# vfdev-5/interpolate-antialiasing

Measured on AMD Instinct MI355X. Metric: Mpix/s (input pixels) antialiased bilinear 438x906->196x320, uint8 channels_last, PIL-exact, higher is better.
Workload: dtype u8; 1 GPU; uint8 channels_last [1024,3,438,906]->[196,320] bilinear antialias per GPU (BASELINE configs[1] batched), Pillow-exact integer arithmetic; batch_per_gpu=1024, global_batch=1024, variant=fused_u8_nhwc_pil_v3, parallelism=batch-shard x1, lib=interpolate_antialiasing_amd/csrc/libaa_interp.so

## Files before the change

interpolate_antialiasing_amd/csrc/aa_fused_u8_v3_impl.h:

```cpp

#pragma once
#include <math.h>
#include <stdio.h>
#include <stdlib.h>

#include <type_traits>

#include "aa_alpha.h"
#include "aa_plan.h"

#ifndef AA_V3_ABL
#define AA_V3_ABL 0
#endif

#ifndef AA_V3_AUX
#define AA_V3_AUX 0
#endif

#ifndef AA_V3_PRIO
#define AA_V3_PRIO 0
#endif
#ifndef AA_V3_DMA_EARLY
#define AA_V3_DMA_EARLY 0
#endif

#ifndef AA_V3_BURST
#define AA_V3_BURST 1
#endif

#ifndef AA_V3_F32OUT_AUX
#define AA_V3_F32OUT_AUX 0
#endif

#ifndef AA_V3_FLT_FAST
#define AA_V3_FLT_FAST 0
#endif

#ifndef AA_V3_UNALIGNED
#define AA_V3_UNALIGNED 0
#endif

struct FusedU8V3Params {
  int H, W, oH, oW;
  int ksize_w, ksize_h;
  int ybands, nstrips;
  int strips_per_block;
  int strip_w;
  int nseg;
  int seg_bytes;
  int sc_off;
  int gather_off;
  int in_mis;
  unsigned long long img_in_bytes, img_out_bytes, total_in_bytes, total_out_bytes;
  long long n_images;
  int spb_forced;
  int outm, normalize, cin;
  float mean[4], std[4];
  unsigned row_pitch;
  int fast;
  int byte_store;
  unsigned long long plane_in_bytes, plane_out_bytes;
  long long pl_planes;
  int out16, pair_store;
};

namespace {

typedef __attribute__((address_space(3))) void lds_void;

#ifndef AA_V3_STORE_AUX
#define AA_V3_STORE_AUX 2
#endif
constexpr int kStoreAuxInterleaved = AA_V3_STORE_AUX;



__device__ inline unsigned pack4_clip8(int a0, int a1, int a2, int a3) {
  unsigned d;
  asm("v_ashr_pk_u8_i32 %0, %1, %2, 22\n\tv_ashr_pk_u8_i32 %0, %3, %4, 22 op_sel:[0,0,0,1]"
      : "=&v"(d)
      : "v"(a0), "v"(a1), "v"(a2), "v"(a3));
  return d;
}

__device__ inline unsigned pack2_bf16(float lo, float hi) {
  unsigned d;
  asm("v_cvt_pk_bf16_f32 %0, %1, %2" : "=v"(d) : "v"(lo), "v"(hi));
  return d;
}
__device__ inline unsigned pack2_f16(float lo, float hi) {
  typedef _Float16 half2_t __attribute__((ext_vector_type(2)));
  const half2_t t = {(_Float16)lo, (_Float16)hi};
  return __builtin_bit_cast(unsigned, t);
}

__device__ inline float right_neighbour(float x) {
  return __int_as_float(__builtin_amdgcn_update_dpp(__float_as_int(x), __float_as_int(x), 0xF5 , 0xF, 0xF, false));
}

__device__ inline int clip8_int(int acc) {
  acc >>= 22;
  return acc < 0 ? 0 : (acc > 255 ? 255 : acc);
}

__device__ inline void wait_vmcnt(int n) {
  if (n >= 12) { asm volatile("s_waitcnt vmcnt(12)" ::: "memory"); return; }
  if (n >= 8) { asm volatile("s_waitcnt vmcnt(8)" ::: "memory"); return; }
  if (n >= 6) { asm volatile("s_waitcnt vmcnt(6)" ::: "memory"); return; }
  if (n >= 4) { asm volatile("s_waitcnt vmcnt(4)" ::: "memory"); return; }
  if (n >= 3) { asm volatile("s_waitcnt vmcnt(3)" ::: "memory"); return; }
  if (n >= 2) { asm volatile("s_waitcnt vmcnt(2)" ::: "memory"); return; }
  if (n >= 1) { asm volatile("s_waitcnt vmcnt(1)" ::: "memory"); return; }
  asm volatile("s_waitcnt vmcnt(0)" ::: "memory");
}

#ifndef AA_V3_WAVES_PER_EU
#define AA_V3_WAVES_PER_EU 0
#endif
#if AA_V3_WAVES_PER_EU
#define AA_V3_OCC __attribute__((amdgpu_waves_per_eu(AA_V3_WAVES_PER_EU, AA_V3_WAVES_PER_EU)))
#else
#define AA_V3_OCC
#endif
template <int C, int TW, int G, bool TWO_DMA, int MAXC, bool NONNEG, bool PERIODIC, bool FLT = false, int UPK = 0, int PL = 0, int SP = 1,
          bool ALPHA = false, bool O16 = false>
__global__ void __launch_bounds__(512) AA_V3_OCC
fused_u8_nhwc_v3_kernel(const uint8_t *__restrict__ in, uint8_t *__restrict__ out, const char *__restrict__ tab_w,
                        const char *__restrict__ tab_h, const FusedU8V3Params p) {
  static_assert(PL == 0 || (PL == C && !PERIODIC && UPK == 0 && !TWO_DMA), "plane groups: shrinking heights, fixed stage layout");
  static_assert(SP == 1 || (SP == 4 && !FLT && !PERIODIC && UPK == 0 && PL == 0), "split windows: integer arithmetic, shrinking heights");
  static_assert(!ALPHA || (C == 4 && !FLT && PL == 0), "premultiplied alpha: Pillow arithmetic, 4 interleaved channels");
  static_assert(!O16 || (FLT && SP == 1), "16-bit float output: float arithmetic");
  constexpr int PLN = PL > 0 ? PL : 1;
  constexpr int CB = PL > 0 ? 1 : C;
  constexpr int NV1 = (CB * TW + 3) / 4;
  constexpr int ND1 = NV1 + 1;
  constexpr int NV = PLN * NV1, ND = PLN * ND1;
  struct SA { unsigned s[PLN]; };
  constexpr int PL_SLOT = 1024, PL_PIECES = 21, PL_PLANE = PL_PIECES * 16;
  extern __shared__ __attribute__((aligned(16))) uint8_t lds[];

  const int lane = threadIdx.x & 63;
  const int wv = __builtin_amdgcn_readfirstlane(threadIdx.x >> 6);
  const int sgroups = (p.nstrips + p.strips_per_block - 1) / p.strips_per_block;
  const int xcd = blockIdx.x & 7, k = blockIdx.x >> 3;
  const int strip = (k % sgroups) * p.strips_per_block + wv;
  const long long grp = (long long)(k / sgroups) * 8 + xcd;
  if (grp >= p.n_images * p.ybands) return;
  if (strip >= p.nstrips) return;
  const bool full_group = (k % sgroups + 1) * p.strips_per_block <= p.nstrips;
  const int yb = (int)(grp % p.ybands);
  const int n = (int)(grp / p.ybands);
  const int ox0 = strip * p.strip_w;
  const int bw = min(p.strip_w, p.oW - ox0);
  const int oy0 = (int)((long long)yb * p.oH / p.ybands);
  const int oy1 = (int)((long long)(yb + 1) * p.oH / p.ybands);

  const int32_t *__restrict__ xmin_w = (const int32_t *)(tab_w + aa_table_xmin_off());
  const int32_t *__restrict__ xsize_w = (const int32_t *)(tab_w + aa_table_xsize_off(p.oW));
  const int32_t *__restrict__ kw = (const int32_t *)(tab_w + aa_table_w_off(p.oW));
  const int32_t *__restrict__ ymin_h = (const int32_t *)(tab_h + aa_table_xmin_off());
  const int32_t *__restrict__ ysize_h = (const int32_t *)(tab_h + aa_table_xsize_off(p.oH));
  const int32_t *__restrict__ sc_rec = (const int32_t *)(tab_h + p.sc_off);
  const int32_t *__restrict__ g_rec = (const int32_t *)(tab_h + p.gather_off);

  const int r_begin = __builtin_amdgcn_readfirstlane(ymin_h[oy0]);
  const int ylm = __builtin_amdgcn_readfirstlane(ymin_h[oy1 - 1]);
  const int yls = __builtin_amdgcn_readfirstlane(ysize_h[oy1 - 1]);
  const int r_stop = ylm + (yls > 1 ? yls : 1);
  const int n_rows = r_stop - r_begin;
  const int n_groups = (n_rows + G - 1) / G;

  const int sp_px = SP > 1 ? lane / SP : lane;
  const int sp_part = SP > 1 ? lane % SP : 0;
  const bool active = sp_px < bw;
  const int ox = ox0 + (active ? sp_px : 0);
  const int xm = xmin_w[ox];
  int xs = xsize_w[ox];
  xs = xs > 1 ? xs : 1;
  int lead = xm + TW * SP - p.W;
  lead = lead > 0 ? lead : 0;
  const int start = xm - lead + sp_part * TW;
  const int acc_init = (SP > 1 && sp_part != 0) ? 0 : 1 << 21;
  int wreg[TW];
#pragma unroll
  for (int j = 0; j < TW; j++) {
    const int src = sp_part * TW + j - lead;
    int w = (src >= 0 && src < xs && src < p.ksize_w) ? kw[(size_t)ox * p.ksize_w + src] : 0;
    wreg[j] = FLT ? w : (w << 8) >> 8;
  }
  asm volatile("s_waitcnt vmcnt(0)" ::: "memory");
  const int seg_first = __builtin_amdgcn_readfirstlane(start * CB);
  const int c_l = start * CB - seg_first;

  const unsigned long long img_off = (unsigned long long)p.in_mis + (unsigned long long)n * p.img_in_bytes;
  const unsigned long long base_off = img_off & ~15ull;
  unsigned long long remaining = p.total_in_bytes - base_off;
  if constexpr (PL == 0) remaining = (remaining + 3ull) & ~3ull;
  if (remaining > 0xFFFFFFFCull) remaining = 0xFFFFFFFCull;
  const __amdgpu_buffer_rsrc_t rsrc =
      __builtin_amdgcn_make_buffer_rsrc((void *)(in + base_off), 0, (unsigned)remaining, 0x00020000);
  const unsigned row_bytes = p.row_pitch;
  const int lds_base = PL > 0 ? wv * G * PL_SLOT : wv * G * p.seg_bytes;
  const unsigned lane_lds = (unsigned)(lds_base + c_l);
  unsigned pl_voff = 0;
  bool pl_dma_lane = false;
  if constexpr (PL > 0) {
    const int pc = lane / PL_PIECES, piece = lane - pc * PL_PIECES;
    pl_voff = (unsigned)pc * (unsigned)p.plane_in_bytes + (unsigned)piece * 16u;
    pl_dma_lane = pc < PL && piece < p.nseg;
  }
  const bool dma_lane0 = PL > 0 ? pl_dma_lane : lane < p.nseg;
  const bool dma_lane1 = lane + 64 < p.nseg;
  constexpr int dma_per_row = TWO_DMA ? 2 : 1;
  const unsigned voff = (unsigned)lane * 16u;

  const unsigned long long out_off = (unsigned long long)n * p.img_out_bytes;
  unsigned long long out_rem = p.total_out_bytes - out_off;
  if (out_rem > 0xFFFFFFFFull) out_rem = 0xFFFFFFFFull;
  const __amdgpu_buffer_rsrc_t orsrc = __builtin_amdgcn_make_buffer_rsrc((void *)(out + out_off), 0, (unsigned)out_rem, 0x00020000);
  const unsigned out_row_bytes = (unsigned)p.oW * CB;
  const int pl_valid = PL > 0 ? (int)(p.pl_planes - (long long)n * PL < PL ? p.pl_planes - (long long)n * PL : PL) : C;
  float nm_mean[C], nm_std[C];
#pragma unroll
  for (int c = 0; c < C; c++) {
    const int ch = PL > 0 ? (int)(((long long)n * PL + c) % (p.cin > 0 ? p.cin : 1))
                          : (C == 1 ? (int)(n % (p.cin > 0 ? p.cin : 1)) : c);
    nm_mean[c] = FLT ? p.mean[ch & 3] : 0.f;
    nm_std[c] = FLT ? p.std[ch & 3] : 1.f;
  }
  unsigned store_voff;
  bool store_lane;
  unsigned perm_sel = 0;
  if constexpr (PL > 0) {
    store_voff = (unsigned)(ox0 + lane);
    store_lane = ((lane & 3) == 0) && ((lane | 3) < bw);
  } else if constexpr (C == 3) {
    const int q = lane & 3;
    store_voff = (unsigned)(ox0 * 3 + (lane >> 2) * 12 + q * 4);
    store_lane = (q != 3) && ((lane | 3) < bw);
    perm_sel = q == 0 ? 0x04020100u : (q == 1 ? 0x05040201u : 0x06050402u);
  } else if constexpr (C == 1) {
    store_voff = (unsigned)(ox0 + lane);
    store_lane = ((lane & 3) == 0) && ((lane | 3) < bw);
  } else {
    store_voff = (unsigned)((ox0 + lane) * 4);
    store_lane = active;
  }

  unsigned a = (unsigned)(img_off - base_off) + (unsigned)seg_first + (unsigned)r_begin * row_bytes;

  int A[MAXC][C];
#pragma unroll
  for (int k = 0; k < MAXC; k++)
#pragma unroll
    for (int c = 0; c < C; c++) A[k][c] = FLT ? 0 : 1 << 21;
  int o_base = oy0;

  constexpr int RK = UPK > 0 ? UPK : 1;
  int ring[RK][C];
#pragma unroll
  for (int k = 0; k < RK; k++)
#pragma unroll
    for (int c = 0; c < C; c++) ring[k][c] = 0;
  int vm_issued = 0, idxv = 0;

  auto dma = [&](unsigned a_row, int slot) {
    if (AA_V3_ABL == 4) return;
    if constexpr (UPK > 0) {
      vm_issued += TWO_DMA ? 2 : 1;
      idxv = (lane == slot) ? vm_issued : idxv;
    }
    if (AA_V3_PRIO) __builtin_amdgcn_s_setprio(3);
    const unsigned soff = AA_V3_ABL == 7 ? (a_row & 0x3F0u) : (a_row & ~15u);
    const int dst = lds_base + slot * (PL > 0 ? PL_SLOT : p.seg_bytes);
    if constexpr (PL > 0) {
      if (dma_lane0) __builtin_amdgcn_raw_ptr_buffer_load_lds(rsrc, (lds_void *)(lds + dst), 16, pl_voff, a_row, 0, AA_V3_AUX);
      if (AA_V3_PRIO) __builtin_amdgcn_s_setprio(0);
      return;
    }
    if (dma_lane0) __builtin_amdgcn_raw_ptr_buffer_load_lds(rsrc, (lds_void *)(lds + dst), 16, voff, soff, 0, AA_V3_AUX);
    if constexpr (TWO_DMA) {
      if (dma_lane1)
        __builtin_amdgcn_raw_ptr_buffer_load_lds(rsrc, (lds_void *)(lds + dst + 1024), 16, voff + 1024, soff, 0, AA_V3_AUX);
    }
    if (AA_V3_PRIO) __builtin_amdgcn_s_setprio(0);
  };
  unsigned slot_ra[G];
  unsigned slot_ph[G];
#pragma unroll
  for (int j = 0; j < G; j++) {
    const unsigned ph = (a + (unsigned)j * row_bytes) & 15u;
    slot_ph[j] = (unsigned)(j * p.seg_bytes) + ph;
    slot_ra[j] = (lane_lds + slot_ph[j]) & ~3u;
  }
  auto fetch = [&](unsigned a_row, int slot, unsigned (&d)[ND], bool tables = true) -> SA {
    SA r;
    unsigned sa, ra;
    if (AA_V3_ABL == 6) { for (int c = 0; c < PLN; c++) r.s[c] = 0; return r; }
    if constexpr (PL > 0) {
      const __attribute__((address_space(3))) unsigned *al = (const __attribute__((address_space(3))) unsigned *)(uintptr_t)(lane_lds & ~3u);
#pragma unroll
      for (int c = 0; c < PL; c++) {
#pragma unroll
        for (int k = 0; k < ND1; k++) d[c * ND1 + k] = al[(slot * PL_SLOT + c * PL_PLANE) / 4 + k];
        r.s[c] = lane_lds;
      }
      return r;
    }
    if (PERIODIC && tables) {
      sa = lane_lds + slot_ph[slot];
      ra = slot_ra[slot];
    } else {
      sa = lane_lds + (unsigned)(slot * p.seg_bytes) + (a_row & 15u);
      ra = sa & ~3u;
    }
    if constexpr (AA_V3_UNALIGNED) {
      typedef unsigned u32_any __attribute__((aligned(1)));
      const __attribute__((address_space(3))) u32_any *ul = (const __attribute__((address_space(3))) u32_any *)(uintptr_t)sa;
#pragma unroll
      for (int k = 0; k < NV; k++) d[k] = ul[k];
      d[ND - 1] = 0;
      r.s[0] = sa;
      return r;
    }
    const __attribute__((address_space(3))) unsigned *al = (const __attribute__((address_space(3))) unsigned *)(uintptr_t)ra;
#pragma unroll
    for (int k = 0; k < ND; k++) d[k] = al[k];
    r.s[0] = sa;
    return r;
  };
  struct Scatter { int first; int cc; int w[MAXC]; };
  auto load_scatter = [&](int r) -> Scatter {
    Scatter s;
    if constexpr (UPK > 0) {
      s.first = 0; s.cc = 0;
#pragma unroll
      for (int k = 0; k < MAXC; k++) s.w[k] = 0;
      return s;
    }
    const int32_t *rec = (const int32_t *)((const char *)sc_rec + (unsigned)r * 32u);
    s.first = __builtin_amdgcn_readfirstlane(rec[0]);
    s.cc = __builtin_amdgcn_readfirstlane(rec[1]);
#pragma unroll
    for (int k = 0; k < MAXC; k++) s.w[k] = __builtin_amdgcn_readfirstlane(rec[2 + k]);
    return s;
  };
  auto trunc8 = [&](int bits) -> unsigned {
    float a = __int_as_float(bits);
    a = a < 0.f ? 0.f : (a > 255.f ? 255.f : a);
    return (unsigned)(int)a;
  };
  const int emit_path = __builtin_amdgcn_readfirstlane(
      (FLT && p.outm != 0) ? (O16 ? (1 | (p.pair_store ? 2 : 0) | (p.out16 == 2 ? 4 : 0) | ((C == 1 || p.outm == 1) ? 8 : 0)) : 1) : (p.byte_store ? 2 : 0));
  auto emit = [&](int oy) {
    if constexpr (ALPHA) {
      const int al = clip8_int(A[0][3]);
#pragma unroll
      for (int c = 0; c < 3; c++) A[0][c] = aa_unpremul8(clip8_int(A[0][c]), al) << 22;
      A[0][3] = al << 22;
    }
    if constexpr (FLT) {
      if constexpr (O16) {
        if (emit_path & 1) {
          int lane_o = lane;
          asm volatile("" : "+v"(lane_o));
          auto pack2 = [&](float lo, float hi) -> unsigned { return (emit_path & 4) ? pack2_bf16(lo, hi) : pack2_f16(lo, hi); };
          auto value = [&](int c) -> float {
            const float x = __int_as_float(A[0][c]);
            return p.normalize ? (x - nm_mean[c]) / nm_std[c] : x;
          };
          const bool pairs = (emit_path & 2) != 0;
          const bool all = lane_o < bw, st = all && (!pairs || (lane_o & 1) == 0);
          if (emit_path & 8) {
            if constexpr (UPK > 0) vm_issued += C;
            const unsigned fv = (unsigned)(ox0 + lane_o) * 2u;
#pragma unroll
            for (int c = 0; c < C; c++) {
              const unsigned fs = ((unsigned)c * (unsigned)p.oH + (unsigned)oy) * (unsigned)p.oW * 2u;
              const float x = value(c);
              const unsigned d = pack2(x, right_neighbour(x));
              if (pairs) {
                if (st && (PL == 0 || c < pl_valid)) __builtin_amdgcn_raw_buffer_store_b32(d, orsrc, fv, fs, AA_V3_F32OUT_AUX);
              } else {
                if (st && (PL == 0 || c < pl_valid)) __builtin_amdgcn_raw_buffer_store_b16((unsigned short)d, orsrc, fv, fs, AA_V3_F32OUT_AUX);
              }
            }
          } else if constexpr (C > 1) {
            const unsigned fv = (unsigned)(ox0 + lane_o) * (unsigned)(2 * C), fs = (unsigned)oy * (unsigned)p.oW * (unsigned)(2 * C);
            float x[C];
#pragma unroll
            for (int c = 0; c < C; c++) x[c] = value(c);
            unsigned d[3];
            if constexpr (C == 3) {
              d[2] = pack2(right_neighbour(x[1]), right_neighbour(x[2]));
              d[1] = pack2(x[2], right_neighbour(x[0]));
              d[0] = pack2(x[0], x[1]);
            } else {
              d[0] = pack2(x[0], x[1]);
              d[1] = pack2(x[2], x[C - 1]);
              d[2] = 0;
            }
            if (!pairs) {
              if constexpr (UPK > 0) vm_issued += C;
#pragma unroll
              for (int c = 0; c < C; c++)
                if (all) __builtin_amdgcn_raw_buffer_store_b16((unsigned short)(d[c >> 1] >> (16 * (c & 1))), orsrc, fv + 2u * (unsigned)c, fs, AA_V3_F32OUT_AUX);
            } else {
              if constexpr (UPK > 0) vm_issued += 1;
              if constexpr (C == 3) {
                typedef unsigned u32x3 __attribute__((ext_vector_type(3)));
                const u32x3 t = {d[0], d[1], d[2]};
                if (st) __builtin_amdgcn_raw_buffer_store_b96(t, orsrc, fv, fs, AA_V3_F32OUT_AUX);
              } else {
                typedef unsigned u32x2 __attribute__((ext_vector_type(2)));
                const u32x2 t = {d[0], d[1]};
                if (all) __builtin_amdgcn_raw_buffer_store_b64(t, orsrc, fv, fs, AA_V3_F32OUT_AUX);
              }
            }
          }
        }
      } else
      if (emit_path == 1) {
        float v[C];
        int lane_o = lane;
        asm volatile("" : "+v"(lane_o));
#pragma unroll
        for (int c = 0; c < C; c++) {
          v[c] = __int_as_float(A[0][c]);
          if (p.normalize) v[c] = (v[c] - nm_mean[c]) / nm_std[c];
        }
        if (p.outm == 1) {
          if constexpr (UPK > 0) vm_issued += C;
#pragma unroll
          for (int c = 0; c < C; c++)
            if (active && (PL == 0 || c < pl_valid))
              __builtin_amdgcn_raw_buffer_store_b32(__float_as_uint(v[c]), orsrc, (unsigned)(ox0 + lane_o) * 4u,
                                                    ((unsigned)c * (unsigned)p.oH + (unsigned)oy) * (unsigned)p.oW * 4u, AA_V3_F32OUT_AUX);
        } else {
          if constexpr (UPK > 0) vm_issued += 1;
          const unsigned fv = (unsigned)(ox0 + lane_o) * (unsigned)(4 * C), fs = (unsigned)oy * (unsigned)p.oW * (unsigned)(4 * C);
          if constexpr (C == 3) {
            typedef unsigned u32x3 __attribute__((ext_vector_type(3)));
            const u32x3 t = {__float_as_uint(v[0]), __float_as_uint(v[1]), __float_as_uint(v[2])};
            if (active) __builtin_amdgcn_raw_buffer_store_b96(t, orsrc, fv, fs, AA_V3_F32OUT_AUX);
          } else if constexpr (C == 4) {
            typedef unsigned u32x4 __attribute__((ext_vector_type(4)));
            const u32x4 t = {__float_as_uint(v[0]), __float_as_uint(v[1]), __float_as_uint(v[2]), __float_as_uint(v[3])};
            if (active) __builtin_amdgcn_raw_buffer_store_b128(t, orsrc, fv, fs, AA_V3_F32OUT_AUX);
          } else {
            if (active) __builtin_amdgcn_raw_buffer_store_b32(__float_as_uint(v[0]), orsrc, fv, fs, AA_V3_F32OUT_AUX);
          }
        }
      }
    }
    if (emit_path == 2) {
      int lane_o = lane;
      asm volatile("" : "+v"(lane_o));
      const int px_o = SP > 1 ? lane_o / SP : lane_o;
      const unsigned bv = (unsigned)((ox0 + px_o) * CB);
      const bool act = px_o < bw && (SP == 1 || (lane_o % SP) == 0);
      if constexpr (UPK > 0) vm_issued += C;
#pragma unroll
      for (int c = 0; c < C; c++) {
        const unsigned b = FLT ? trunc8(A[0][c]) : (unsigned)clip8_int(A[0][c]);
        if constexpr (PL > 0) {
          if (act && c < pl_valid) __builtin_amdgcn_raw_buffer_store_b8((unsigned char)b, orsrc, bv, (unsigned)c * (unsigned)p.plane_out_bytes + (unsigned)oy * out_row_bytes, 0);
        } else {
          if (act) __builtin_amdgcn_raw_buffer_store_b8((unsigned char)b, orsrc, bv + c, (unsigned)oy * out_row_bytes, 0);
        }
      }
    }
    if constexpr (UPK > 0) {
      if (emit_path == 0) vm_issued += 1;
    }
    if (emit_path != 0) {
    } else if constexpr (PL > 0) {
      const unsigned t = FLT ? (trunc8(A[0][0]) | (trunc8(A[0][1]) << 8) | (trunc8(A[0][PL > 2 ? 2 : 1]) << 16))
                             : pack4_clip8(A[0][0], A[0][1], A[0][PL > 2 ? 2 : 1], A[0][PL - 1]);
      const unsigned nb = (unsigned)__builtin_amdgcn_update_dpp(0, (int)t, 0xF5 , 0xF, 0xF, false);
#pragma unroll
      for (int c = 0; c < PL; c++) {
        const unsigned pair = __builtin_amdgcn_perm(nb, t, 0x0c0c0000u | (unsigned)((4 + c) << 8) | (unsigned)c);
        const unsigned hi = (unsigned)__builtin_amdgcn_update_dpp(0, (int)pair, 0xAA , 0xF, 0xF, false);
        const unsigned dw = __builtin_amdgcn_perm(hi, pair, 0x05040100u);
        if (store_lane && c < pl_valid) __builtin_amdgcn_raw_buffer_store_b32(dw, orsrc, store_voff, (unsigned)c * (unsigned)p.plane_out_bytes + (unsigned)oy * out_row_bytes, 0);
      }
    } else if constexpr (C == 3) {
      const unsigned t = FLT ? (trunc8(A[0][0]) | (trunc8(A[0][1]) << 8) | (trunc8(A[0][2]) << 16))
                             : pack4_clip8(A[0][0], A[0][1], A[0][2], A[0][2]);
      const unsigned nb = (unsigned)__builtin_amdgcn_update_dpp(0, (int)t, 0xF9 , 0xF, 0xF, false);
      const unsigned dw = __builtin_amdgcn_perm(nb, t, perm_sel);
      if (store_lane && (AA_V3_ABL != 1 || dw == 0x12345678u))
        __builtin_amdgcn_raw_buffer_store_b32(dw, orsrc, store_voff, AA_V3_ABL == 9 ? 0u : (unsigned)oy * out_row_bytes, C == 1 ? 0 : kStoreAuxInterleaved);
    } else if constexpr (C == 1) {
      const unsigned t = FLT ? trunc8(A[0][0]) * 0x01010101u : pack4_clip8(A[0][0], A[0][0], A[0][0], A[0][0]);
      const unsigned n1 = (unsigned)__builtin_amdgcn_update_dpp(0, (int)t, 0x55 , 0xF, 0xF, false);
      const unsigned n2 = (unsigned)__builtin_amdgcn_update_dpp(0, (int)t, 0xAA , 0xF, 0xF, false);
      const unsigned n3 = (unsigned)__builtin_amdgcn_update_dpp(0, (int)t, 0xFF , 0xF, 0xF, false);
      const unsigned dw = (t & 0x000000ffu) | (n1 & 0x0000ff00u) | (n2 & 0x00ff0000u) | (n3 & 0xff000000u);
      if (store_lane) __builtin_amdgcn_raw_buffer_store_b32(dw, orsrc, store_voff, (unsigned)oy * out_row_bytes, C == 1 ? 0 : kStoreAuxInterleaved);
    } else {
      const unsigned dw = FLT ? (trunc8(A[0][0]) | (trunc8(A[0][1]) << 8) | (trunc8(A[0][2]) << 16) | (trunc8(A[0][C - 1]) << 24))
                              : pack4_clip8(A[0][0], A[0][1], A[0][2], A[0][C - 1]);
      if (store_lane) __builtin_amdgcn_raw_buffer_store_b32(dw, orsrc, store_voff, (unsigned)oy * out_row_bytes, C == 1 ? 0 : kStoreAuxInterleaved);
    }
#pragma unroll
    for (int k = 0; k + 1 < MAXC; k++)
#pragma unroll
      for (int c = 0; c < C; c++) A[k][c] = A[k + 1][c];
#pragma unroll
    for (int c = 0; c < C; c++) A[MAXC - 1][c] = FLT ? 0 : 1 << 21;
  };
  struct GRow { int m; int s; int w[RK]; };
  auto load_grow = [&](int oy) -> GRow {
    GRow gr;
    const int o = oy < p.oH ? oy : p.oH - 1;
    const int32_t *rec = (const int32_t *)((const char *)g_rec + (unsigned)o * 32u);
    gr.m = __builtin_amdgcn_readfirstlane(rec[0]);
    gr.s = __builtin_amdgcn_readfirstlane(rec[1]);
#pragma unroll
    for (int k = 0; k < RK; k++) gr.w[k] = __builtin_amdgcn_readfirstlane(rec[2 + (k < 6 ? k : 5)]);
    return gr;
  };
  GRow g_cur, g_nxt;
  if constexpr (UPK > 0) {
    g_cur = load_grow(oy0);
    g_nxt = load_grow(oy0 + 1);
  }
  int r = r_begin;
  auto realign = [&](const unsigned (&d)[ND], const SA &sa, unsigned (&v)[NV]) {
#pragma unroll
    for (int c = 0; c < PLN; c++)
#pragma unroll
      for (int k = 0; k < NV1; k++)
        v[c * NV1 + k] = AA_V3_UNALIGNED ? d[c * ND1 + k] : __builtin_amdgcn_alignbyte(d[c * ND1 + k + 1], d[c * ND1 + k], sa.s[c]);
  };
  bool steady = false;
  auto row_step = [&](const unsigned (&v)[NV], const Scatter &sc, auto steady_tag) {
    constexpr bool STEADY = decltype(steady_tag)::value;
    if (AA_V3_ABL == 6) return;
    int h[C];
    if constexpr (FLT) {
      float accf[C];
#pragma unroll
      for (int j = 0; j < TW; j++) {
#pragma unroll
        for (int c = 0; c < C; c++) {
          const int bi = PL > 0 ? c * (4 * NV1) + j : j * C + c;
          const float px = (float)((v[bi >> 2] >> (8 * (bi & 3))) & 0xffu);
          if constexpr (AA_V3_FLT_FAST != 0) {
            accf[c] = j == 0 ? px * __int_as_float(wreg[j]) : __builtin_fmaf(px, __int_as_float(wreg[j]), accf[c]);
            continue;
          }
          const float prod = px * __int_as_float(wreg[j]);
          accf[c] = j == 0 ? prod : accf[c] + prod;
        }
      }
#pragma unroll
      for (int c = 0; c < C; c++) h[c] = __float_as_int(accf[c]);
    } else {
      int acc[C];
#pragma unroll
      for (int c = 0; c < C; c++) acc[c] = AA_V3_ABL == 5 ? (int)v[c] : (SP > 1 ? acc_init : 1 << 21);
#pragma unroll
      for (int j = 0; j < (AA_V3_ABL == 5 ? 0 : TW); j++) {
#pragma unroll
        for (int c = 0; c < C; c++) {
          const int bi = PL > 0 ? c * (4 * NV1) + j : j * C + c;
          int px = (int)((v[bi >> 2] >> (8 * (bi & 3))) & 0xffu);
          if constexpr (ALPHA) {
            if (c < 3) px = aa_premul8(px, (int)(v[j] >> 24));
          }
          acc[c] += px * wreg[j];
        }
      }
      if constexpr (SP > 1) {
#pragma unroll
        for (int c = 0; c < C; c++) {
          acc[c] += __builtin_amdgcn_update_dpp(0, acc[c], 0xB1 , 0xF, 0xF, false);
          acc[c] += __builtin_amdgcn_update_dpp(0, acc[c], 0x4E , 0xF, 0xF, false);
        }
      }
#pragma unroll
      for (int c = 0; c < C; c++) h[c] = NONNEG ? (int)((unsigned)acc[c] >> 22) : clip8_int(acc[c]);
    }
    if constexpr (UPK > 0) {
#pragma unroll
      for (int k = 0; k + 1 < RK; k++)
#pragma unroll
        for (int c = 0; c < C; c++) ring[k][c] = ring[k + 1][c];
#pragma unroll
      for (int c = 0; c < C; c++) ring[RK - 1][c] = h[c];
      while (o_base < oy1) {
        int gs = g_cur.s > 1 ? g_cur.s : 1;
        if (g_cur.m + gs != r + 1) break;
        gs = gs < RK ? gs : RK;
#pragma unroll
        for (int ss = 1; ss <= RK; ss++) {
          if (gs == ss) {
#pragma unroll
            for (int c = 0; c < C; c++) {
              int acc;
              if constexpr (FLT) {
                float f = __int_as_float(ring[RK - ss][c]) * __int_as_float(g_cur.w[0]);
#pragma unroll
                for (int k2 = 1; k2 < ss; k2++) f = f + __int_as_float(ring[RK - ss + k2][c]) * __int_as_float(g_cur.w[k2]);
                acc = __float_as_int(f);
              } else {
                acc = (1 << 21) + __mul24(ring[RK - ss][c], g_cur.w[0]);
#pragma unroll
                for (int k2 = 1; k2 < ss; k2++) acc += __mul24(ring[RK - ss + k2][c], g_cur.w[k2]);
              }
              A[0][c] = acc;
            }
          }
        }
        emit(o_base);
        o_base++;
        g_cur = g_nxt;
        g_nxt = load_grow(o_base + 1);
      }
      return;
    }
    auto vmac = [&](int a, int hv, int w) -> int {
      if constexpr (FLT && AA_V3_FLT_FAST != 0) return __float_as_int(__builtin_fmaf(__int_as_float(hv), __int_as_float(w), __int_as_float(a)));
      else if constexpr (FLT) return __float_as_int(__int_as_float(a) + __int_as_float(hv) * __int_as_float(w));
      else return a + __mul24(hv, w);
    };
    const int idx0 = sc.first - o_base;
    if constexpr (STEADY) {
#pragma unroll
      for (int k = 0; k < MAXC; k++) {
        if (k >= 2 && k >= (sc.cc & 0xFFFF)) break;
#pragma unroll
        for (int c = 0; c < C; c++) A[k][c] = vmac(A[k][c], h[c], sc.w[k]);
      }
    } else if (__builtin_expect(idx0 == 0, 1)) {
      steady = true;
#pragma unroll
      for (int k = 0; k < MAXC; k++) {
        if (k >= 2 && k >= (sc.cc & 0xFFFF)) break;
#pragma unroll
        for (int c = 0; c < C; c++) A[k][c] = vmac(A[k][c], h[c], sc.w[k]);
      }
    } else if (idx0 < 0 && idx0 > -MAXC) {
#pragma unroll
      for (int s = 1; s < MAXC; s++) {
        if (idx0 == -s) {
#pragma unroll
          for (int k = s; k < MAXC; k++)
#pragma unroll
            for (int c = 0; c < C; c++) A[k - s][c] = vmac(A[k - s][c], h[c], sc.w[k]);
        }
      }
    }
    const int sc_end = sc.first + (sc.cc >> 16);
    const int e_end = sc_end < oy1 ? sc_end : oy1;
    while (o_base < e_end) {
      emit(o_base);
      o_base++;
    }
  };

  const int pl_fix_row = (PL > 0 && (long long)n + 1 == p.n_images) ? p.H - 1 : -1;
  auto pl_patch_last = [&](int slot) {
    if constexpr (PL > 0) {
      const int q = p.W - 3 + lane;
      const int lpos = q - seg_first;
      if (lane < 3 && q >= 0 && lpos >= 0 && lpos < p.nseg * 16) {
        const uint8_t b = in[img_off + (unsigned long long)(pl_valid - 1) * p.plane_in_bytes + (unsigned long long)(p.H - 1) * row_bytes + (unsigned)q];
        lds[lds_base + slot * PL_SLOT + (pl_valid - 1) * PL_PLANE + lpos] = b;
      }
      asm volatile("s_waitcnt vmcnt(0) lgkmcnt(0)" ::: "memory");
    }
  };

  for (int i = 0; i < G; i++)
    if (i < n_rows) dma(a + (unsigned)i * row_bytes, i);
  unsigned d0[ND], d1[ND];
  SA sa0 = {}, sa1 = {};
  Scatter sc0 = load_scatter(r_begin), sc1 = sc0;
  {
    const int younger = (n_rows < G ? n_rows : G) - 1;
    wait_vmcnt(younger * dma_per_row);
    if (PL > 0 && r_begin == pl_fix_row) pl_patch_last(0);
    sa0 = fetch(a, 0, d0, false);
  }
  for (int g = 0; g < n_groups; g++) {
    const int x0 = g * G;
    auto unrolled_group = [&](auto steady_tag) {
      if (full_group) __builtin_amdgcn_s_barrier();
#pragma unroll
      for (int i = 0; i < G; i++) {
        if (AA_V3_ABL != 2) asm volatile("s_waitcnt vmcnt(%0)" ::"n"(dma_per_row * (G - 2 - (i % AA_V3_BURST))) : "memory");
        unsigned v[NV];
        if ((i & 1) == 0) {
          realign(d0, sa0, v);
          __builtin_amdgcn_sched_barrier(0);
          sc1 = load_scatter(r + 1);
          sa1 = fetch(a + row_bytes, (i + 1) % G, d1);
          __builtin_amdgcn_sched_barrier(0);
          if (AA_V3_DMA_EARLY) { dma(a + (unsigned)G * row_bytes, i); __builtin_amdgcn_sched_barrier(0); }
          row_step(v, sc0, steady_tag);
        } else {
          realign(d1, sa1, v);
          __builtin_amdgcn_sched_barrier(0);
          sc0 = load_scatter(r + 1);
          sa0 = fetch(a + row_bytes, (i + 1) % G, d0);
          __builtin_amdgcn_sched_barrier(0);
          if (AA_V3_DMA_EARLY) { dma(a + (unsigned)G * row_bytes, i); __builtin_amdgcn_sched_barrier(0); }
          row_step(v, sc1, steady_tag);
        }
        if (!AA_V3_DMA_EARLY) {
          if constexpr (AA_V3_BURST == 1) {
            dma(a + (unsigned)G * row_bytes, i);
          } else if ((i % AA_V3_BURST) == AA_V3_BURST - 1) {
#pragma unroll
            for (int b = AA_V3_BURST - 1; b >= 0; b--) dma(a + (unsigned)(G - b) * row_bytes, i - b);
          }
        }
        a += row_bytes;
        r++;
        __builtin_amdgcn_sched_barrier(0);
      }
    };
    if (UPK == 0 && x0 + 2 * G <= n_rows) {
      if (steady) unrolled_group(std::true_type{});
      else unrolled_group(std::false_type{});
    } else {
      for (int i = 0; i < G; i++) {
        const int x = x0 + i;
        if (x >= n_rows) break;
        if (x + 1 < n_rows) {
          if constexpr (UPK > 0) {
            const int my_idx = __builtin_amdgcn_readlane(idxv, __builtin_amdgcn_readfirstlane((i + 1) % G));
            wait_vmcnt(vm_issued - my_idx);
          } else {
            int younger = n_rows - 1 - (x + 1);
            younger = younger < G - 2 ? younger : G - 2;
            wait_vmcnt(younger * dma_per_row);
          }
          if (PL > 0 && r + 1 == pl_fix_row) pl_patch_last((i + 1) % G);
          if ((i & 1) == 0) { sc1 = load_scatter(r + 1); sa1 = fetch(a + row_bytes, (i + 1) % G, d1, false); }
          else { sc0 = load_scatter(r + 1); sa0 = fetch(a + row_bytes, (i + 1) % G, d0, false); }
        }
        unsigned v[NV];
        if ((i & 1) == 0) { realign(d0, sa0, v); row_step(v, sc0, std::false_type{}); }
        else { realign(d1, sa1, v); row_step(v, sc1, std::false_type{}); }
        if (x + G < n_rows) dma(a + (unsigned)G * row_bytes, i);
        a += row_bytes;
        r++;
      }
    }
  }
}

int pick_ybands(int64_t items_per_band, double slots, int taps_h, int64_t H, int64_t oH) {
  const int64_t max_yb = oH / 8 > 1 ? oH / 8 : 1;
  int64_t ybands = 1;
  double best = 1e30;
  for (int64_t yb = 1; yb <= max_yb && yb <= 64; yb++) {
    const double rounds = (double)items_per_band * yb / slots;
    const double eff = rounds / ceil(rounds);
    const double halo = 1.0 + (double)(yb - 1) * taps_h / (double)H;
    const double cost = halo / eff;
    if (cost < best - 1e-9) {
      best = cost;
      ybands = yb;
    }
  }
  if (const char *e = aa_knob("AA_FUSED_YBANDS")) {
    const int64_t v = atoll(e);
    if (v >= 1 && v <= max_yb) ybands = v;
  }
  return (int)ybands;
}

template <int C, int TW, int G, int MAXC, bool TWO, bool NONNEG, bool PERIODIC, bool FLT = false, int UPK = 0, int PL = 0, int SP = 1,
          bool ALPHA = false, bool O16 = false>
int launch_k(FusedU8V3Params p, const AAProblem &q, size_t lds) {
  auto kern = fused_u8_nhwc_v3_kernel<C, TW, G, TWO, MAXC, NONNEG, PERIODIC, FLT, UPK, PL, SP, ALPHA, O16>;
  auto resident = [&](int s) {
    int nb = aa_resident_blocks(kern, 64 * s, lds * s);
    if (nb <= 0) nb = 16 / s;
    return nb < 1 ? 1 : nb;
  };
  int spb = p.strips_per_block;
  if (spb > 1 && !p.spb_forced && resident(1) > resident(spb) * spb) spb = 1;
  p.strips_per_block = spb;
  const int sgroups = (p.nstrips + spb - 1) / spb;
  const size_t lds_blk = lds * spb;
  const int taps_h = q.ah.max_taps > 0 ? q.ah.max_taps : q.ah.ksize;
  p.ybands = pick_ybands(p.n_images * sgroups, (double)aa_device_cu_count() * resident(spb), taps_h, q.H, q.oH);
  if (aa_knob("AA_V3_DEBUG"))
    fprintf(stderr, "[aa v3] strips %d spb %d (resident(1) %d, resident(%d) %d) ybands %d lds/strip %zu images %lld\n", p.nstrips, spb,
            resident(1), p.nstrips <= 8 ? p.nstrips : 4, resident(p.nstrips <= 8 ? p.nstrips : 4), p.ybands, lds, (long long)p.n_images);
  const int64_t groups8 = (p.n_images * (int64_t)p.ybands + 7) / 8 * 8;
  const int64_t grid = groups8 * sgroups;
  if (grid > 0x7FFFFFFF) return 0;
  hipLaunchKernelGGL(kern, dim3((unsigned)grid), dim3(64 * spb), lds_blk,
                     q.stream, (const uint8_t *)q.in - p.in_mis, (uint8_t *)q.out, (const char *)q.aw.table_dev,
                     (const char *)q.ah.table_dev, p);
  AA_HIP_CHECK_LAUNCH();
  return 1;
}

int round_tw(int taps) {
  const int opts[] = {2, 4, 6, 8, 12, 16, 24, 34};
  for (int o : opts)
    if (taps <= o) return o;
  return 0;
}

}

enum V3Route {
#define V3_ROUTE(route, ...) V3_##route,
#include "aa_fused_u8_v3_list.h"
};
enum V3Arith { V3_PIL = 1, V3_FLT = 2, V3_BOTH = 3 };
constexpr bool v3_route_has_out16(int route) { return route == V3_NARROW || route == V3_UP || route == V3_PLANES; }
```

Baseline: 1.405 million Mpix/s.

## Replace accumulator sliding with parity-indexed double accumulators and dword-only emit path

Result: slower. 1.379 million Mpix/s (-1.8%).

```diff
diff --git a/interpolate_antialiasing_amd/csrc/aa_fused_u8_v3_impl.h b/interpolate_antialiasing_amd/csrc/aa_fused_u8_v3_impl.h
--- a/interpolate_antialiasing_amd/csrc/aa_fused_u8_v3_impl.h
+++ b/interpolate_antialiasing_amd/csrc/aa_fused_u8_v3_impl.h
@@ -38,6 +38,10 @@
 
 #ifndef AA_V3_UNALIGNED
 #define AA_V3_UNALIGNED 0
+#endif
+
+#ifndef AA_V3_NOSLIDE
+#define AA_V3_NOSLIDE 1
 #endif
 
 struct FusedU8V3Params {
@@ -98,6 +102,10 @@
   return __int_as_float(__builtin_amdgcn_update_dpp(__float_as_int(x), __float_as_int(x), 0xF5 , 0xF, 0xF, false));
 }
 
+template <int QUAD_PERM> __device__ inline unsigned quad_move(unsigned x) {
+  return (unsigned)__builtin_amdgcn_mov_dpp((int)x, QUAD_PERM, 0xF, 0xF, true);
+}
+
 __device__ inline int clip8_int(int acc) {
   acc >>= 22;
   return acc < 0 ? 0 : (acc > 255 ? 255 : acc);
@@ -353,21 +361,27 @@
   };
   const int emit_path = __builtin_amdgcn_readfirstlane(
       (FLT && p.outm != 0) ? (O16 ? (1 | (p.pair_store ? 2 : 0) | (p.out16 == 2 ? 4 : 0) | ((C == 1 || p.outm == 1) ? 8 : 0)) : 1) : (p.byte_store ? 2 : 0));
-  auto emit = [&](int oy) {
+  constexpr bool NS = AA_V3_NOSLIDE != 0 && MAXC == 2 && !FLT && UPK == 0 && PL == 0 && SP == 1 && !ALPHA;
+  int par = 0;
+  auto emit = [&](int oy, auto set_tag, auto dw_tag) {
+    constexpr int S = decltype(set_tag)::value;
+    constexpr bool DW = decltype(dw_tag)::value;
+    static_assert(S == 0 || NS, "only the no-slide form emits from a set other than 0");
+    static_assert(!DW || !FLT, "the dword-only form belongs to the Pillow-arithmetic kernels");
     if constexpr (ALPHA) {
-      const int al = clip8_int(A[0][3]);
-#pragma unroll
-      for (int c = 0; c < 3; c++) A[0][c] = aa_unpremul8(clip8_int(A[0][c]), al) << 22;
-      A[0][3] = al << 22;
-    }
-    if constexpr (FLT) {
+      const int al = clip8_int(A[S][3]);
+#pragma unroll
+      for (int c = 0; c < 3; c++) A[S][c] = aa_unpremul8(clip8_int(A[S][c]), al) << 22;
+      A[S][3] = al << 22;
+    }
+    if constexpr (FLT && !DW) {
       if constexpr (O16) {
         if (emit_path & 1) {
           int lane_o = lane;
           asm volatile("" : "+v"(lane_o));
           auto pack2 = [&](float lo, float hi) -> unsigned { return (emit_path & 4) ? pack2_bf16(lo, hi) : pack2_f16(lo, hi); };
           auto value = [&](int c) -> float {
-            const float x = __int_as_float(A[0][c]);
+            const float x = __int_as_float(A[S][c]);
             return p.normalize ? (x - nm_mean[c]) / nm_std[c] : x;
           };
           const bool pairs = (emit_path & 2) != 0;
@@ -427,7 +441,7 @@
         asm volatile("" : "+v"(lane_o));
 #pragma unroll
         for (int c = 0; c < C; c++) {
-          v[c] = __int_as_float(A[0][c]);
+          v[c] = __int_as_float(A[S][c]);
           if (p.normalize) v[c] = (v[c] - nm_mean[c]) / nm_std[c];
         }
         if (p.outm == 1) {
@@ -454,7 +468,7 @@
         }
       }
     }
-    if (emit_path == 2) {
+    if (!DW && emit_path == 2) {
       int lane_o = lane;
       asm volatile("" : "+v"(lane_o));
       const int px_o = SP > 1 ? lane_o / SP : lane_o;
@@ -463,7 +477,7 @@
       if constexpr (UPK > 0) vm_issued += C;
 #pragma unroll
       for (int c = 0; c < C; c++) {
-        const unsigned b = FLT ? trunc8(A[0][c]) : (unsigned)clip8_int(A[0][c]);
+        const unsigned b = FLT ? trunc8(A[S][c]) : (unsigned)clip8_int(A[S][c]);
         if constexpr (PL > 0) {
           if (act && c < pl_valid) __builtin_amdgcn_raw_buffer_store_b8((unsigned char)b, orsrc, bv, (unsigned)c * (unsigned)p.plane_out_bytes + (unsigned)oy * out_row_bytes, 0);
         } else {
@@ -474,43 +488,48 @@
     if constexpr (UPK > 0) {
       if (emit_path == 0) vm_issued += 1;
     }
-    if (emit_path != 0) {
+    if (!DW && emit_path != 0) {
     } else if constexpr (PL > 0) {
-      const unsigned t = FLT ? (trunc8(A[0][0]) | (trunc8(A[0][1]) << 8) | (trunc8(A[0][PL > 2 ? 2 : 1]) << 16))
-                             : pack4_clip8(A[0][0], A[0][1], A[0][PL > 2 ? 2 : 1], A[0][PL - 1]);
-      const unsigned nb = (unsigned)__builtin_amdgcn_update_dpp(0, (int)t, 0xF5 , 0xF, 0xF, false);
+      const unsigned t = FLT ? (trunc8(A[S][0]) | (trunc8(A[S][1]) << 8) | (trunc8(A[S][PL > 2 ? 2 : 1]) << 16))
+                             : pack4_clip8(A[S][0], A[S][1], A[S][PL > 2 ? 2 : 1], A[S][PL - 1]);
+      const unsigned nb = quad_move<0xF5>(t) ;
 #pragma unroll
       for (int c = 0; c < PL; c++) {
         const unsigned pair = __builtin_amdgcn_perm(nb, t, 0x0c0c0000u | (unsigned)((4 + c) << 8) | (unsigned)c);
-        const unsigned hi = (unsigned)__builtin_amdgcn_update_dpp(0, (int)pair, 0xAA , 0xF, 0xF, false);
+        const unsigned hi = quad_move<0xAA>(pair) ;
         const unsigned dw = __builtin_amdgcn_perm(hi, pair, 0x05040100u);
         if (store_lane && c < pl_valid) __builtin_amdgcn_raw_buffer_store_b32(dw, orsrc, store_voff, (unsigned)c * (unsigned)p.plane_out_bytes + (unsigned)oy * out_row_bytes, 0);
       }
     } else if constexpr (C == 3) {
-      const unsigned t = FLT ? (trunc8(A[0][0]) | (trunc8(A[0][1]) << 8) | (trunc8(A[0][2]) << 16))
-                             : pack4_clip8(A[0][0], A[0][1], A[0][2], A[0][2]);
-      const unsigned nb = (unsigned)__builtin_amdgcn_update_dpp(0, (int)t, 0xF9 , 0xF, 0xF, false);
+      const unsigned t = FLT ? (trunc8(A[S][0]) | (trunc8(A[S][1]) << 8) | (trunc8(A[S][2]) << 16))
+                             : pack4_clip8(A[S][0], A[S][1], A[S][2], A[S][2]);
+      const unsigned nb = quad_move<0xF9>(t) ;
       const unsigned dw = __builtin_amdgcn_perm(nb, t, perm_sel);
       if (store_lane && (AA_V3_ABL != 1 || dw == 0x12345678u))
         __builtin_amdgcn_raw_buffer_store_b32(dw, orsrc, store_voff, AA_V3_ABL == 9 ? 0u : (unsigned)oy * out_row_bytes, C == 1 ? 0 : kStoreAuxInterleaved);
     } else if constexpr (C == 1) {
-      const unsigned t = FLT ? trunc8(A[0][0]) * 0x01010101u : pack4_clip8(A[0][0], A[0][0], A[0][0], A[0][0]);
-      const unsigned n1 = (unsigned)__builtin_amdgcn_update_dpp(0, (int)t, 0x55 , 0xF, 0xF, false);
-      const unsigned n2 = (unsigned)__builtin_amdgcn_update_dpp(0, (int)t, 0xAA , 0xF, 0xF, false);
-      const unsigned n3 = (unsigned)__builtin_amdgcn_update_dpp(0, (int)t, 0xFF , 0xF, 0xF, false);
+      const unsigned t = FLT ? trunc8(A[S][0]) * 0x01010101u : pack4_clip8(A[S][0], A[S][0], A[S][0], A[S][0]);
+      const unsigned n1 = quad_move<0x55>(t) ;
+      const unsigned n2 = quad_move<0xAA>(t) ;
+      const unsigned n3 = quad_move<0xFF>(t) ;
       const unsigned dw = (t & 0x000000ffu) | (n1 & 0x0000ff00u) | (n2 & 0x00ff0000u) | (n3 & 0xff000000u);
       if (store_lane) __builtin_amdgcn_raw_buffer_store_b32(dw, orsrc, store_voff, (unsigned)oy * out_row_bytes, C == 1 ? 0 : kStoreAuxInterleaved);
     } else {
-      const unsigned dw = FLT ? (trunc8(A[0][0]) | (trunc8(A[0][1]) << 8) | (trunc8(A[0][2]) << 16) | (trunc8(A[0][C - 1]) << 24))
-                              : pack4_clip8(A[0][0], A[0][1], A[0][2], A[0][C - 1]);
+      const unsigned dw = FLT ? (trunc8(A[S][0]) | (trunc8(A[S][1]) << 8) | (trunc8(A[S][2]) << 16) | (trunc8(A[S][C - 1]) << 24))
+                              : pack4_clip8(A[S][0], A[S][1], A[S][2], A[S][C - 1]);
       if (store_lane) __builtin_amdgcn_raw_buffer_store_b32(dw, orsrc, store_voff, (unsigned)oy * out_row_bytes, C == 1 ? 0 : kStoreAuxInterleaved);
     }
-#pragma unroll
-    for (int k = 0; k + 1 < MAXC; k++)
-#pragma unroll
-      for (int c = 0; c < C; c++) A[k][c] = A[k + 1][c];
-#pragma unroll
-    for (int c = 0; c < C; c++) A[MAXC - 1][c] = FLT ? 0 : 1 << 21;
+    if constexpr (NS) {
+#pragma unroll
+      for (int c = 0; c < C; c++) A[S][c] = 1 << 21;
+    } else {
+#pragma unroll
+      for (int k = 0; k + 1 < MAXC; k++)
+#pragma unroll
+        for (int c = 0; c < C; c++) A[k][c] = A[k + 1][c];
+#pragma unroll
+      for (int c = 0; c < C; c++) A[MAXC - 1][c] = FLT ? 0 : 1 << 21;
+    }
   };
   struct GRow { int m; int s; int w[RK]; };
   auto load_grow = [&](int oy) -> GRow {
@@ -537,7 +556,7 @@
         v[c * NV1 + k] = AA_V3_UNALIGNED ? d[c * ND1 + k] : __builtin_amdgcn_alignbyte(d[c * ND1 + k + 1], d[c * ND1 + k], sa.s[c]);
   };
   bool steady = false;
-  auto row_step = [&](const unsigned (&v)[NV], const Scatter &sc, auto steady_tag) {
+  auto row_step = [&](const unsigned (&v)[NV], const Scatter &sc, auto steady_tag, auto dw_tag) {
     constexpr bool STEADY = decltype(steady_tag)::value;
     if (AA_V3_ABL == 6) return;
     int h[C];
@@ -616,7 +635,7 @@
             }
           }
         }
-        emit(o_base);
+        emit(o_base, std::integral_constant<int, 0>{}, dw_tag);
         o_base++;
         g_cur = g_nxt;
         g_nxt = load_grow(o_base + 1);
@@ -629,7 +648,19 @@
       else return a + __mul24(hv, w);
     };
     const int idx0 = sc.first - o_base;
-    if constexpr (STEADY) {
+    if constexpr (NS) {
+      int lw0 = sc.w[0], lw1 = sc.w[1];
+      if constexpr (!STEADY) {
+        if (idx0 == 0) steady = true;
+        lw0 = idx0 == 0 ? sc.w[0] : (idx0 == -1 ? sc.w[1] : 0);
+        lw1 = idx0 == 0 ? sc.w[1] : 0;
+      }
+      const int pw0 = par ? lw1 : lw0, pw1 = par ? lw0 : lw1;
+#pragma unroll
+      for (int c = 0; c < C; c++) A[0][c] = vmac(A[0][c], h[c], pw0);
+#pragma unroll
+      for (int c = 0; c < C; c++) A[1][c] = vmac(A[1][c], h[c], pw1);
+    } else if constexpr (STEADY) {
 #pragma unroll
       for (int k = 0; k < MAXC; k++) {
         if (k >= 2 && k >= (sc.cc & 0xFFFF)) break;
@@ -657,9 +688,20 @@
     }
     const int sc_end = sc.first + (sc.cc >> 16);
     const int e_end = sc_end < oy1 ? sc_end : oy1;
-    while (o_base < e_end) {
-      emit(o_base);
-      o_base++;
+    if constexpr (NS) {
+#pragma unroll
+      for (int k = 0; k < MAXC; k++) {
+        if (o_base >= e_end) break;
+        if (par) emit(o_base, std::integral_constant<int, 1>{}, dw_tag);
+        else emit(o_base, std::integral_constant<int, 0>{}, dw_tag);
+        par ^= 1;
+        o_base++;
+      }
+    } else {
+      while (o_base < e_end) {
+        emit(o_base, std::integral_constant<int, 0>{}, dw_tag);
+        o_base++;
+      }
     }
   };
 
@@ -689,7 +731,7 @@
   }
   for (int g = 0; g < n_groups; g++) {
     const int x0 = g * G;
-    auto unrolled_group = [&](auto steady_tag) {
+    auto unrolled_group = [&](auto steady_tag, auto dw_tag) {
       if (full_group) __builtin_amdgcn_s_barrier();
 #pragma unroll
       for (int i = 0; i < G; i++) {
@@ -702,7 +744,7 @@
           sa1 = fetch(a + row_bytes, (i + 1) % G, d1);
           __builtin_amdgcn_sched_barrier(0);
           if (AA_V3_DMA_EARLY) { dma(a + (unsigned)G * row_bytes, i); __builtin_amdgcn_sched_barrier(0); }
-          row_step(v, sc0, steady_tag);
+          row_step(v, sc0, steady_tag, dw_tag);
         } else {
           realign(d1, sa1, v);
           __builtin_amdgcn_sched_barrier(0);
@@ -710,7 +752,7 @@
           sa0 = fetch(a + row_bytes, (i + 1) % G, d0);
           __builtin_amdgcn_sched_barrier(0);
           if (AA_V3_DMA_EARLY) { dma(a + (unsigned)G * row_bytes, i); __builtin_amdgcn_sched_barrier(0); }
-          row_step(v, sc1, steady_tag);
+          row_step(v, sc1, steady_tag, dw_tag);
         }
         if (!AA_V3_DMA_EARLY) {
           if constexpr (AA_V3_BURST == 1) {
@@ -726,8 +768,16 @@
       }
     };
     if (UPK == 0 && x0 + 2 * G <= n_rows) {
-      if (steady) unrolled_group(std::true_type{});
-      else unrolled_group(std::false_type{});
+      const bool dw_only = !FLT && emit_path == 0;
+      if (dw_only) {
+        if constexpr (!FLT) {
+          if (steady) unrolled_group(std::true_type{}, std::true_type{});
+          else unrolled_group(std::false_type{}, std::true_type{});
+        }
+      } else {
+        if (steady) unrolled_group(std::true_type{}, std::false_type{});
+        else unrolled_group(std::false_type{}, std::false_type{});
+      }
     } else {
       for (int i = 0; i < G; i++) {
         const int x = x0 + i;
@@ -746,8 +796,8 @@
           else { sc0 = load_scatter(r + 1); sa0 = fetch(a + row_bytes, (i + 1) % G, d0, false); }
         }
         unsigned v[NV];
-        if ((i & 1) == 0) { realign(d0, sa0, v); row_step(v, sc0, std::false_type{}); }
-        else { realign(d1, sa1, v); row_step(v, sc1, std::false_type{}); }
+        if ((i & 1) == 0) { realign(d0, sa0, v); row_step(v, sc0, std::false_type{}, std::false_type{}); }
+        else { realign(d1, sa1, v); row_step(v, sc1, std::false_type{}, std::false_type{}); }
         if (x + G < n_rows) dma(a + (unsigned)G * row_bytes, i);
         a += row_bytes;
         r++;
```
